# dpfried/action-segmentation

Measured on AMD Instinct MI355X. Metric: frames/sec semi-Markov decode, CrossTask T~10k K~20 L=1024, 1/2/4/8 GPUs, higher is better.
Workload: dtype f64

## Files before the change

### action-segmentation_amd/_build.py

```python
import os
import shutil
import subprocess
from concurrent.futures import ThreadPoolExecutor

HERE = os.path.dirname(os.path.abspath(__file__))
CSRC = os.path.join(HERE, "csrc")
OBJ = os.path.join(CSRC, "_obj")
LIB = os.path.join(HERE, "libsmmdp.so")
SOURCES = ["smm_api.hip", "smm_emission.hip", "smm_viterbi.hip", "smm_chunk.hip", "smm_logz.hip", "smm_logz_bwd.hip", "smm_dense.hip",
           "smm_eval.hip", "smm_fit.hip", "smm_tables.hip", "smm_sample.hip", "smm_kbest.hip",
           "smm_entropy.hip", "smm_kl.hip", "smm_entropy_bwd.hip", "smm_mbr.hip", "smm_align.hip", "smm_align_opt.hip", "smm_align_logz.hip",
           "smm_align_opt_logz.hip", "smm_align_graph.hip", "smm_align_graph_logz.hip",
           "smm_align_graph_sample.hip", "smm_align_graph_entropy.hip", "smm_align_graph_kl.hip",
           "smm_align_graph_entropy_bwd.hip"]
HEADERS = ["smm_device.h", "smm_launch.h", "smm_align_tile.h", "smm_align_lse.h", "smm_align_graph.h", "smm_posterior.h", "smm_draw.h", "smm_plan_feedback.h", os.path.join("..", "..", "include", "smmdp.h")]
FLAGS = ["--offload-arch=gfx950", "-O3", "-ffp-contract=off", "-fPIC", "-std=c++17",
         "-mllvm", "-pragma-unroll-threshold=1048576", "-mllvm", "-unroll-threshold=1048576"]


UNIT_FLAGS = {"smm_viterbi.hip": ["-fno-honor-nans", "-DSMM_FMAX_BUILTIN"]}


def _extra_flags():
    return os.environ.get("SMM_DEV_FLAGS", "").split()


def _obj(src):
    return os.path.join(OBJ, os.path.splitext(src)[0] + ".o")


def _stale_obj(src, force):
    o = _obj(src)
    if force or not os.path.exists(o):
        return True
    t = os.path.getmtime(o)
    return any(os.path.getmtime(os.path.join(CSRC, f)) > t for f in [src] + HEADERS)


def stale():
    if not os.path.exists(LIB):
        return True
    t = os.path.getmtime(LIB)
    return any(os.path.getmtime(os.path.join(CSRC, f)) > t for f in SOURCES + HEADERS)


def build(force=False, verbose=False):
    if not force and not stale():
        return LIB
# ... 57 lines not shown
```

### action-segmentation_amd/_lib.py

```python
import ctypes
import os

HERE = os.path.dirname(os.path.abspath(__file__))
LIB_PATH = os.environ.get("SMM_LIB_PATH") or os.path.join(HERE, "libsmmdp.so")

SYMBOLS = [
    "smm_strerror", "smm_last_hip_error", "smm_version", "smm_device_count", "smm_workspace_bytes",
    "smm_error_word_offset", "smm_dp_timing_enable", "smm_dp_timing_read", "smm_dp_timing_read_tagged", "smm_band_frame_ns", "smm_time_split_plan",
    "smm_env_reload", "smm_release_cached_plans", "smm_cached_plan_bytes", "smm_plan_feedback_info", "smm_plan_feedback_plan",
    "smm_emission_f64", "smm_emission_bwd_f64", "smm_viterbi_f64", "smm_viterbi_f32", "smm_decode_f32", "smm_logz_f64", "smm_logz_bwd_f64",
    "smm_sample_f64", "smm_entropy_f64", "smm_kl_f64", "smm_kbest_workspace_bytes", "smm_kbest_f64",
    "smm_mbr_workspace_bytes", "smm_mbr_f64",
    "smm_align_workspace_bytes", "smm_align_f64", "smm_align_opt_workspace_bytes", "smm_align_opt_f64",
    "smm_align_graph_workspace_bytes", "smm_align_graph_f64",
    "smm_align_logz_workspace_bytes", "smm_align_logz_f64", "smm_align_logz_bwd_f64",
    "smm_align_opt_logz_workspace_bytes", "smm_align_opt_logz_f64", "smm_align_opt_logz_bwd_f64",
    "smm_align_graph_logz_workspace_bytes", "smm_align_graph_logz_f64", "smm_align_graph_logz_bwd_f64",
    "smm_align_graph_sample_f64", "smm_align_graph_entropy_f64", "smm_align_graph_kl_f64",
    "smm_entropy_bwd_scratch_bytes", "smm_entropy_bwd_f64", "smm_kl_bwd_f64",
    "smm_align_graph_entropy_bwd_scratch_bytes", "smm_align_graph_entropy_bwd_f64", "smm_align_graph_kl_bwd_f64",
    "smm_factor_tables_f64", "smm_factor_tables_bwd_f64",
    "smm_dense_workspace_bytes", "smm_dense_dp_f32", "smm_dense_marginals_f32",
    "smm_eval_workspace_bytes", "smm_eval_confusion_i64", "smm_eval_videos_i64",
    "smm_fit_workspace_bytes", "smm_fit_error_word_offset", "smm_fit_stats_f64",
]


class SmmShape(ctypes.Structure):
    _fields_ = [("b", ctypes.c_int32), ("d", ctypes.c_int32), ("n_groups", ctypes.c_int32),
                ("c_max", ctypes.c_int32), ("k_rows", ctypes.c_int32), ("t_max", ctypes.c_int32),
                ("flags", ctypes.c_int32), ("total_frames", ctypes.c_int64)]


class SmmPlanFeedbackInfo(ctypes.Structure):
    _fields_ = [("n_replans", ctypes.c_int32), ("n1_before", ctypes.c_int32), ("n1_after", ctypes.c_int32),
                ("n_videos", ctypes.c_int32), ("end_before_us", ctypes.c_double), ("end_after_us", ctypes.c_double),
                ("stamps", ctypes.POINTER(ctypes.c_uint64)), ("order", ctypes.POINTER(ctypes.c_int32))]


class SmmTablesShape(ctypes.Structure):
    _fields_ = [("n_classes", ctypes.c_int32), ("d", ctypes.c_int32), ("n_groups", ctypes.c_int32),
# ... 114 lines not shown
                                                                                         ctypes.c_void_p]
    lib.smm_error_word_offset.argtypes = [ctypes.POINTER(SmmShape)]
    lib.smm_kl_f64.restype = ctypes.c_int
    lib.smm_kl_f64.argtypes = [ctypes.POINTER(SmmShape)] + [ctypes.c_void_p] * 11 + [ctypes.c_void_p, ctypes.c_size_t] \
        + [ctypes.c_void_p] * 6 + [ctypes.c_void_p, ctypes.c_size_t] + [ctypes.c_void_p] * 3
    lib.smm_entropy_bwd_scratch_bytes.restype = ctypes.c_size_t
    lib.smm_entropy_bwd_scratch_bytes.argtypes = [ctypes.POINTER(SmmShape), ctypes.c_void_p]
    lib.smm_entropy_bwd_f64.restype = ctypes.c_int
    lib.smm_entropy_bwd_f64.argtypes = [ctypes.POINTER(SmmShape)] + [ctypes.c_void_p] * 17 + [ctypes.c_void_p, ctypes.c_size_t] \
        + [ctypes.c_void_p, ctypes.c_size_t, ctypes.c_void_p]
    lib.smm_kl_bwd_f64.restype = ctypes.c_int
    lib.smm_kl_bwd_f64.argtypes = [ctypes.POINTER(SmmShape)] + [ctypes.c_void_p] * 11 + [ctypes.c_void_p, ctypes.c_size_t] \
        + [ctypes.c_void_p] * 6 + [ctypes.c_void_p, ctypes.c_size_t, ctypes.c_int32] + [ctypes.c_void_p] * 6 \
        + [ctypes.c_void_p, ctypes.c_size_t, ctypes.c_void_p]
    lib.smm_align_graph_entropy_bwd_scratch_bytes.restype = ctypes.c_size_t
    lib.smm_align_graph_entropy_bwd_scratch_bytes.argtypes = [ctypes.POINTER(SmmShape), ctypes.c_void_p, ctypes.c_void_p]
    lib.smm_align_graph_entropy_bwd_f64.restype = ctypes.c_int
    lib.smm_align_graph_entropy_bwd_f64.argtypes = [ctypes.POINTER(SmmShape)] + [ctypes.c_void_p] * 21 \
        + [ctypes.c_void_p, ctypes.c_size_t] * 2 + [ctypes.c_void_p]
    lib.smm_align_graph_kl_bwd_f64.restype = ctypes.c_int
    lib.smm_align_graph_kl_bwd_f64.argtypes = [ctypes.POINTER(SmmShape)] + [ctypes.c_void_p] * 11 + [ctypes.c_void_p, ctypes.c_size_t] \
        + [ctypes.c_void_p] * 4 + [ctypes.c_void_p, ctypes.c_size_t] + [ctypes.c_void_p] * 4 + [ctypes.c_int32] \
        + [ctypes.c_void_p] * 6 + [ctypes.c_void_p, ctypes.c_size_t, ctypes.c_void_p]
    lib.smm_dp_timing_enable.restype = None
    lib.smm_dp_timing_enable.argtypes = [ctypes.c_int]
    lib.smm_dp_timing_read.restype = ctypes.c_int
    lib.smm_dp_timing_read.argtypes = [ctypes.POINTER(ctypes.c_float), ctypes.c_int]
    lib.smm_dp_timing_read_tagged.restype = ctypes.c_int
    lib.smm_dp_timing_read_tagged.argtypes = [ctypes.POINTER(ctypes.c_float), ctypes.POINTER(ctypes.c_int32), ctypes.c_int]
    lib.smm_band_frame_ns.restype = ctypes.c_double
    lib.smm_band_frame_ns.argtypes = [ctypes.c_int]
    lib.smm_time_split_plan.restype = ctypes.c_int
    lib.smm_time_split_plan.argtypes = [ctypes.POINTER(SmmShape)] + [ctypes.c_void_p] * 4 + [ctypes.c_int] + [ctypes.c_void_p] * 4 + [ctypes.c_int]
    lib.smm_env_reload.restype = None
    lib.smm_env_reload.argtypes = []
    lib.smm_release_cached_plans.restype = ctypes.c_size_t
    lib.smm_release_cached_plans.argtypes = []
    lib.smm_cached_plan_bytes.restype = ctypes.c_size_t
    lib.smm_cached_plan_bytes.argtypes = []
    lib.smm_plan_feedback_info.restype = ctypes.c_int
    lib.smm_plan_feedback_info.argtypes = [ctypes.POINTER(SmmPlanFeedbackInfo)]
    lib.smm_plan_feedback_plan.restype = ctypes.c_int
    lib.smm_plan_feedback_plan.argtypes = [ctypes.c_int, ctypes.c_int, ctypes.c_double] + [ctypes.c_void_p] * 3 + [ctypes.c_int, ctypes.c_int] \
        + [ctypes.c_void_p] * 4
    _lib = lib
    return lib


def reload_env():
    if _lib is not None:
        _lib.smm_env_reload()


def check(status):
    if status != 0:
        lib = load()
        msg = lib.smm_strerror(status).decode()
        if status == -4:
            msg += " (hipError %d)" % lib.smm_last_hip_error()
        raise SmmError("libsmmdp: %s" % msg)


def host_cores():
    import os
    env = os.environ.get('SMM_HOST_CORES')
    if env:
# ... 17 lines not shown
```

### action-segmentation_amd/csrc/smm_api.hip

```cpp
#include <algorithm>
#include <atomic>
#include <functional>
#include <cstdio>
#include <cstdlib>
#include <cstring>
#include <numeric>
#include <vector>
#include <unordered_map>
#include <mutex>
#include <utility>
#include <string>

#include "../../include/smmdp.h"
#include "smm_device.h"
#include "smm_launch.h"
#include "smm_plan_feedback.h"

static thread_local int g_last_hip = 0;

namespace {
struct SmmEnv {
    int spec = 1;
    int no_split = 0;
    double split_min_us = 100.0, split_ns = 0.0;
    int split_margin = 400;
    int plan_cache = 1;
    int small_wg = 1;
    int plan_feedback = 1;
    int chunk = 1;
    int chunk_p = 0;
    int chunk_lmin = 0;
    int chunk_wc = 512;
    int no_bt_window = 0;
    int fit_grid = 0;
    int verbose = 0;
#ifdef SMM_DEV
    int debug_flags = 0;
    int split_debug = 0;
    int upload_memcpy = 0;
    int emission_v2 = 0;
#endif
    std::string key;
};
std::atomic<const SmmEnv *> g_env{nullptr};
std::once_flag g_env_once;

void env_read()
{
    SmmEnv e;
    struct Item { const char *name; int *i; double *d; };
    const Item items[] = {
        {"SMM_SPEC", &e.spec, nullptr}, {"SMM_NO_SPLIT", &e.no_split, nullptr}, {"SMM_SPLIT_MIN_US", nullptr, &e.split_min_us},
        {"SMM_SPLIT_NS", nullptr, &e.split_ns}, {"SMM_SPLIT_MARGIN", &e.split_margin, nullptr},
        {"SMM_PLAN_CACHE", &e.plan_cache, nullptr}, {"SMM_SMALL_WG", &e.small_wg, nullptr}, {"SMM_PLAN_FEEDBACK", &e.plan_feedback, nullptr}, {"SMM_CHUNK", &e.chunk, nullptr}, {"SMM_CHUNK_P", &e.chunk_p, nullptr},
        {"SMM_CHUNK_WC", &e.chunk_wc, nullptr}, {"SMM_CHUNK_LMIN", &e.chunk_lmin, nullptr}, {"SMM_NO_BT_WINDOW", &e.no_bt_window, nullptr},
        {"SMM_FIT_GRID", &e.fit_grid, nullptr}, {"SMM_VERBOSE", &e.verbose, nullptr},
#ifdef SMM_DEV
        {"SMM_DEBUG_FLAGS", &e.debug_flags, nullptr}, {"SMM_SPLIT_DEBUG", &e.split_debug, nullptr},
        {"SMM_UPLOAD_MEMCPY", &e.upload_memcpy, nullptr}, {"SMM_EMISSION_V2", &e.emission_v2, nullptr},
#endif
    };
    for (const Item &it : items) {
        const char *v = std::getenv(it.name);
        if (!v) continue;
        if (it.i) *it.i = (*v == 0) ? 1 : std::atoi(v);
        if (it.d) *it.d = std::atof(v);
        e.key += it.name; e.key += '='; e.key += v; e.key += ';';
    }
    g_env.store(new SmmEnv(e), std::memory_order_release);
}
const SmmEnv &env()
{
    std::call_once(g_env_once, env_read);
    return *g_env.load(std::memory_order_acquire);
}
}

extern "C" void smm_env_reload(void)
{
    (void)env();
    env_read();
}
int smm_env_fit_grid() { return env().fit_grid; }
int smm_env_emission_v2()
{
#ifdef SMM_DEV
    return env().emission_v2;
#else
// ... 235 lines not shown
    SmmChunkVideo *cvs;
    int32_t *redo;
    double *anchors;
    int n_cv, n_units, u_part1;
    int small_first, small_count;
    uint64_t *stamps = nullptr;
    hipEvent_t done = nullptr;
    void *fb_entry = nullptr;
    std::vector<int32_t> order_host, frames_host;
};

static bool band_mode(int kp_max, int c_need);

static int device_cus()
{
    static std::mutex mu;
    static int n_cu[64] = {};
    int dev = 0;
    if (hipGetDevice(&dev) != hipSuccess || dev < 0 || dev >= 64) return 0;
    std::lock_guard<std::mutex> lock(mu);
    if (!n_cu[dev] && hipDeviceGetAttribute(&n_cu[dev], hipDeviceAttributeMultiprocessorCount, dev) != hipSuccess) n_cu[dev] = 0;
    return n_cu[dev] > 0 ? n_cu[dev] : 0;
}

constexpr double SMM_BAND_NS_BASE = 145.0, SMM_BAND_NS_PER_STATE = 2.0;
extern "C" double smm_band_frame_ns(int n_states)
{
    if (n_states < 1 || n_states > SMM_MAX_STATES) return 0.0;
    return SMM_BAND_NS_BASE + SMM_BAND_NS_PER_STATE * n_states;
}

static double dp_frame_ns(bool band, int c) { return band ? smm_band_frame_ns(c) : 150.0 + 3.0 * c; }

static int choose_split(const SmmVideo *hv, int32_t *order, int b, int d, int c_max, int64_t total_frames)
{
    const SmmEnv &ev = env();
    if (b < 24 || ev.no_split) return 0;
    const int n_cu = device_cus();
    if (n_cu <= 0) return 0;
    const double em_us = (double)total_frames * (4.0 * d + 8.0 * c_max) / 4.0e6;
    if (em_us < ev.split_min_us) return 0;
    int tmax = 0;
    for (int i = 0; i < b; ++i) tmax = std::max(tmax, hv[i].T);
    const double split_ns = ev.split_ns > 0.0 ? ev.split_ns : 1.75 * smm_band_frame_ns(std::min(c_max, (int)SMM_MAX_STATES));
    const int thr = tmax - (int)(em_us * 1000.0 / split_ns) - ev.split_margin;
    int n1 = 0;
    for (int i = 0; i < b; ++i) n1 += hv[i].T >= thr;
    if (thr <= 0 || n1 < 1 || n1 > b / 3 || n1 > n_cu / 2 || b - n1 < 16 || b > 2 * n_cu) return 0;
    std::stable_partition(order, order + b, [&](int32_t v) { return hv[v].T >= thr; });
    return n1;
}

namespace {
struct PlanFeedback {
    uint64_t *stamps = nullptr;
    hipEvent_t done = nullptr;
    bool pending = false;
    bool have = false;
    bool busy = false;
    int evals_left = 5, n_replans = 0;
    int b = 0, n1_first = 0;
    double em_us = 0.0, end_before_us = 0.0, end_after_us = 0.0;
    std::vector<uint64_t> snap, used;
    std::vector<int32_t> order, frames;
};
constexpr int SMM_FEEDBACK_MAX_REPLANS = 4;
constexpr double SMM_FEEDBACK_MIN_GAIN = 0.02;
struct PlanEntry {
    PlanFeedback *fb = nullptr;
    std::vector<char> key;
    int device = 0;
// ... 372 lines not shown
}

extern "C" int smm_plan_feedback_info(smm_plan_feedback_info_t *out)
{
    if (!out) return SMM_ERR_ARG;
    std::lock_guard<std::mutex> lock(g_plans.mu);
    *out = g_fb_info.generation == g_plans.generation ? g_fb_info.info : smm_plan_feedback_info_t{};
    return SMM_OK;
}

extern "C" int smm_plan_feedback_plan(int b, int n_cu, double em_us, const double *dur_us, const int32_t *frames,
                                      const int32_t *cur_order, int cur_n1, int force, int32_t *order_out, int32_t *n1_out,
                                      double *end_current_us, double *end_chosen_us)
{
    if (b < 1 || n_cu < 1 || !dur_us || !frames || !cur_order || cur_n1 < 0 || cur_n1 > b) return SMM_ERR_ARG;
    std::vector<char> seen(b, 0);
    for (int i = 0; i < b; ++i) {
        if (cur_order[i] < 0 || cur_order[i] >= b || seen[cur_order[i]]) return SMM_ERR_ARG;
        seen[cur_order[i]] = 1;
    }
    const SmmFeedbackPlan p = smm_feedback_plan(dur_us, frames, cur_order, b, cur_n1, n_cu, em_us, force != 0);
    if (order_out) std::memcpy(order_out, p.order.data(), sizeof(int32_t) * b);
    if (n1_out) *n1_out = p.n1;
    if (end_current_us) *end_current_us = p.end_current_us;
    if (end_chosen_us) *end_chosen_us = p.end_chosen_us;
    return p.changed ? 1 : 0;
}

struct ChunkPlan {
    std::vector<SmmVideo> units;
    std::vector<SmmChunkVideo> cvs;
};

static void plan_chunks_lmin(const smm_shape *s, const SmmVideo *hv, const int32_t *n_states, int kp_max, bool band, ChunkPlan &out, int n_cu_given, int lmin_cfg)
{
    const SmmEnv &ev = env();
    if (!ev.chunk || (s->flags & (SMM_SHAPE_NO_EOS | SMM_SHAPE_NO_TIME_SPLIT)) || kp_max <= 64) return;
    const int n_cu = n_cu_given > 0 ? n_cu_given : device_cus();
    if (n_cu <= 0) return;
    auto ns = [&](int c) { return dp_frame_ns(band, c); };
    double t_cu = 0.0, t_long = 0.0;
    for (int i = 0; i < s->b; ++i) {
        const double t = (double)hv[i].T * ns(n_states[hv[i].group]);
        t_cu += t;
        t_long = std::max(t_long, t);
    }
    t_cu = t_cu / n_cu + (s->d > 0 ? (double)s->total_frames * (4.0 * s->d + 8.0 * s->c_max) / 4.0e3 : 0.0);
    if (ev.chunk_p <= 0 && t_long < 1.5 * t_cu) return;
    const size_t units_cap = chunk_units_max(s);
    for (int i = 0; i < s->b; ++i) {
        const int T = hv[i].T, C = n_states[hv[i].group], kpv = hv[i].kp;
        const int ov = std::max(std::min(ev.chunk_wc, kpv), 16) + kpv - 1;
        const int lmin = std::max(kpv - 1, std::min(lmin_cfg, 2 * kpv));
        const int pmin = ov + lmin;
        int P = ev.chunk_p > 0 ? ev.chunk_p : (int)(1.1 * t_cu / ns(C));
        P = std::max(P, pmin);
        if ((double)T < 1.05 * P || T < pmin + lmin) continue;
        int n_rest = (T - P + (P - ov) - 1) / (P - ov);
        int Pq = 0;
        for (; n_rest >= 1; --n_rest) {
            Pq = (int)(((int64_t)T + (int64_t)n_rest * ov + n_rest) / (n_rest + 1));
            if (Pq - ov >= lmin) break;
        }
        if (n_rest < 1 || n_rest + 1 > SMM_CHUNK_MAX_UNITS) continue;
        const int L = Pq - ov;
        size_t need = (size_t)3 * C * ((size_t)Pq + 1);
        for (int j = 1; j <= n_rest; ++j) {
            const int r = Pq + (j - 1) * L, e = (j == n_rest) ? T : r + L;
            need += (size_t)3 * C * ((size_t)(e - (r - ov)) + 1);
        }
        if (need > (size_t)8 * s->c_max * ((size_t)T + 1) || Pq + (n_rest - 1) * L >= T) continue;
        if (out.units.size() + n_rest + 1 > units_cap) break;
        SmmChunkVideo cv{i, (int32_t)out.units.size(), n_rest + 1, ov};
        size_t hoff = (size_t)hv[i].hist_off;
        for (int j = 0; j <= n_rest; ++j) {
            const int r = j ? Pq + (j - 1) * L : 0, a0 = j ? r - ov : 0, e = (j == n_rest) ? T : Pq + j * L;
            SmmVideo u = hv[i];
            u.frame_off = hv[i].frame_off + a0;
            u.hist_off = (int64_t)hoff;
            u.T = e - a0;
            u.pad = 1 | (j ? 2 : 0) | (a0 << 2);
            hoff += (size_t)3 * C * ((size_t)u.T + 1);
            out.units.push_back(u);
        }
        out.cvs.push_back(cv);
    }
}

static void plan_chunks(const smm_shape *s, const SmmVideo *hv, const int32_t *n_states, int kp_max, bool band, ChunkPlan &out, int n_cu_given = 0)
{
    const SmmEnv &ev = env();
    if (ev.chunk_lmin > 0) { plan_chunks_lmin(s, hv, n_states, kp_max, band, out, n_cu_given, std::max(ev.chunk_lmin, 130)); return; }
    const int n_cu = n_cu_given > 0 ? n_cu_given : device_cus();
    ChunkPlan fine;
    plan_chunks_lmin(s, hv, n_states, kp_max, band, fine, n_cu_given, SMM_CHUNK_LMIN_FINE);
    if (!fine.cvs.empty() && (int)fine.units.size() + (s->b - (int)fine.cvs.size()) <= n_cu) { out = std::move(fine); return; }
    plan_chunks_lmin(s, hv, n_states, kp_max, band, out, n_cu_given, SMM_CHUNK_LMIN);
}

static int stage_uncached(const smm_shape *s, const int64_t *lengths, const int64_t *frame_off, const int32_t *group,
                          const int32_t *kp, const int32_t *n_states, void *ws, size_t ws_bytes, hipStream_t stream, Staged *out,
                          bool for_viterbi, int cum_chunk, bool want_split, const std::function<char *(size_t)> *meta_alloc,
                          SmmPlan *plan_out)
{
    if (!shape_ok(s) || !lengths || !frame_off || !n_states || !ws) return SMM_ERR_ARG;
    if (!limits_ok(s)) return SMM_ERR_UNSUPPORTED;
    int c_need = 0;
    for (int g = 0; g < s->n_groups; ++g) {
        if (n_states[g] < 1 || n_states[g] > s->c_max) return SMM_ERR_ARG;
        c_need = std::max(c_need, n_states[g]);
    }
    const bool no_eos = (s->flags & SMM_SHAPE_NO_EOS) != 0;
    for (int i = 0; i < s->b; ++i)
        if (lengths[i] < (no_eos ? 2 : 1) || lengths[i] > s->t_max) return SMM_ERR_ARG;
    const SmmPlan p = make_plan(s, lengths);
    if (ws_bytes < p.total) return SMM_ERR_WORKSPACE;

    std::vector<char> host(p.meta_bytes, 0);
    SmmVideo *hv = reinterpret_cast<SmmVideo *>(host.data());
    int32_t *ho = reinterpret_cast<int32_t *>(host.data() + p.o_order);
    int32_t *hn = reinterpret_cast<int32_t *>(host.data() + p.o_nstates);

    size_t hoff = 0;
    int kp_max = 2;
    for (int i = 0; i < s->b; ++i) {
        const int64_t t = lengths[i];
        if (frame_off[i] < 0 || frame_off[i] + t > s->total_frames) return SMM_ERR_ARG;
        const int g = group ? group[i] : 0;
        if (g < 0 || g >= s->n_groups) return SMM_ERR_ARG;
        const int k = kp ? kp[i] : std::min<int>(s->k_rows, s->t_max);
        if (k < 1 || k > s->k_rows) return SMM_ERR_ARG;
        hv[i].frame_off = frame_off[i];
        hv[i].hist_off = (int64_t)hoff;
        hv[i].T = (int32_t)t;
        hv[i].group = g;
        hv[i].kp = k;
        hv[i].pad = 0;
        hoff += 8 * (size_t)s->c_max * (size_t)(t + 1);
        kp_max = std::max(kp_max, k);
    }
    std::iota(ho, ho + s->b, 0);
    out->band_mode = band_mode(kp_max, c_need);
    const bool band = out->band_mode;
    std::stable_sort(ho, ho + s->b, [&](int a, int b) {
        return hv[a].T * dp_frame_ns(band, n_states[hv[a].group]) > hv[b].T * dp_frame_ns(band, n_states[hv[b].group]);
    });
    if (cum_chunk > 0) std::stable_sort(ho, ho + s->b, [&](int a, int b) { return hv[a].group < hv[b].group; });
    std::memcpy(hn, n_states, sizeof(int32_t) * s->n_groups);
    ChunkPlan cp;
    if (for_viterbi && cum_chunk == 0) plan_chunks(s, hv, n_states, kp_max, out->band_mode, cp);
    const int n_cv = (int)cp.cvs.size(), n_un = (int)cp.units.size();
    out->n_cv = n_cv;
    out->n_units = s->b - n_cv + n_un;
    out->u_part1 = n_un;
    out->n_split = 0;
    if (n_cv > 0) {
        std::vector<char> is_cv(s->b, 0);
        for (const SmmChunkVideo &cv : cp.cvs) is_cv[cv.vid] = 1;
        std::stable_partition(ho, ho + s->b, [&](int32_t v) { return is_cv[v] != 0; });
        const SmmEnv &ev = env();
        const double em_us = (double)s->total_frames * (4.0 * s->d + 8.0 * s->c_max) / 4.0e6;
        if (want_split && !ev.no_split && s->b - n_cv >= 16 && em_us >= ev.split_min_us) out->n_split = n_cv;
    } else {
        out->n_split = want_split ? choose_split(hv, ho, s->b, s->d, s->c_max, s->total_frames) : 0;
    }
    out->small_first = out->small_count = 0;
    if (for_viterbi && cum_chunk == 0 && out->band_mode && env().small_wg && !(s->flags & SMM_SHAPE_NO_EOS)) {
        const bool force = env().small_wg >= 2;
        const int n_cu = device_cus();
        const int t0 = out->n_split > 0 ? out->n_split : n_cv;
        const int n_tail = s->b - t0;
        if (n_cu > 0 && (force || n_tail >= 3 * n_cu)) {
            double t_cu = 0.0;
            for (int i = t0; i < s->b; ++i) t_cu += (double)hv[ho[i]].T * smm_band_frame_ns(n_states[hv[ho[i]].group]);
            t_cu /= n_cu;
            auto small = [&](int32_t v) {
                return n_states[hv[v].group] <= 16 && (force || (double)hv[v].T * 1.6 * smm_band_frame_ns(n_states[hv[v].group]) <= 0.5 * t_cu);
            };
            const int n_small = (int)std::count_if(ho + t0, ho + s->b, small);
            if (n_small >= (force ? 1 : 64)) {
                std::stable_partition(ho + t0, ho + s->b, [&](int32_t v) { return !small(v); });
                out->small_count = n_small;
            }
// ... 41 lines not shown
            xp[i] = cp.cvs[i].vid;
        }
    }

    if (out->small_count > 0) out->small_first = out->n_units - out->small_count;

    char *base = static_cast<char *>(ws);
    const size_t o_ext = align_up(p.o_err, 256);
    char *meta_dst = meta_alloc ? (*meta_alloc)(o_ext + ext.size()) : nullptr;
    char *meta = meta_dst ? meta_dst : base;
    SMM_HIP((hipError_t)smm_upload_meta(meta, host.data(), p.o_err, stream));
    SMM_HIP((hipError_t)smm_zero_async(base + p.o_err, p.meta_bytes - p.o_err, stream));
    out->videos = reinterpret_cast<SmmVideo *>(meta);
    out->order = reinterpret_cast<int32_t *>(meta + p.o_order);
    out->n_states = reinterpret_cast<int32_t *>(meta + p.o_nstates);
    out->em_cum = reinterpret_cast<int32_t *>(meta + p.o_emcum);
    plan_point(p, ws, out);
    out->uvideos = nullptr; out->uorder = nullptr; out->porder = nullptr; out->cvs = nullptr;
    if (n_cv > 0) {
        char *xdst = meta_dst ? meta_dst + o_ext
                              : base + p.o_chunk + align_up(sizeof(int32_t) * s->b, 256) + align_up(sizeof(double) * chunk_units_max(s) * s->c_max, 256);
        SMM_HIP((hipError_t)smm_upload_meta(xdst, ext.data(), ext.size(), stream));
        out->uvideos = reinterpret_cast<SmmVideo *>(xdst);
        out->uorder = reinterpret_cast<int32_t *>(xdst + x_order);
        out->cvs = reinterpret_cast<SmmChunkVideo *>(xdst + x_cvs);
        out->porder = reinterpret_cast<int32_t *>(xdst + x_porder);
    }
    out->kp_max = kp_max;
    out->c_need = c_need;
    if (plan_out) *plan_out = p;
    return SMM_OK;
}

extern "C" int smm_time_split_plan(const smm_shape *s, const int64_t *lengths, const int32_t *group, const int32_t *kp,
                                   const int32_t *n_states, int n_cu, int32_t *unit_video, int32_t *unit_first, int32_t *unit_len,
                                   int32_t *unit_overlap, int cap)
{
    if (!shape_ok(s) || !lengths || !n_states || n_cu < 1) return SMM_ERR_ARG;
    std::vector<SmmVideo> hv(s->b);
    size_t hoff = 0;
    int kp_max = 2, c_need = 0;
    for (int g = 0; g < s->n_groups; ++g) c_need = std::max(c_need, n_states[g]);
    for (int i = 0; i < s->b; ++i) {
        const int g = group ? group[i] : 0;
        if (g < 0 || g >= s->n_groups || lengths[i] < 1) return SMM_ERR_ARG;
        hv[i] = SmmVideo{0, (int64_t)hoff, (int32_t)lengths[i], g, kp ? kp[i] : std::min<int>(s->k_rows, s->t_max), 0};
        hoff += 8 * (size_t)s->c_max * (size_t)(lengths[i] + 1);
        kp_max = std::max(kp_max, hv[i].kp);
    }
    ChunkPlan cp;
    plan_chunks(s, hv.data(), n_states, kp_max, band_mode(kp_max, c_need), cp, n_cu);
    int n = 0;
    for (const SmmChunkVideo &cv : cp.cvs)
        for (int j = 0; j < cv.n_chunks; ++j, ++n) {
            if (n >= cap) continue;
            const SmmVideo &u = cp.units[cv.first_unit + j];
            if (unit_video) unit_video[n] = cv.vid;
            if (unit_first) unit_first[n] = u.pad >> 2;
            if (unit_len) unit_len[n] = u.T;
            if (unit_overlap) unit_overlap[n] = j ? cv.ov : 0;
        }
    return n;
}

static bool band_mode(int kp_max, int c_need)
{
    return kp_max > 512 || (kp_max > 256 && c_need > 28);
}

static int ring_regs(int kp_max)
{
    int r = 1;
    while (64 * r < kp_max) r *= 2;
    return r;
}

struct Tables {
    const double *elp, *trans, *init, *len, *endpen, *logz;
};

static SmmDpArgs dp_args(const smm_shape *s, const Staged &st, const Tables &t)
{
    SmmDpArgs a{};
    a.videos = st.videos; a.order = st.order; a.n_states = st.n_states;
    a.elp = t.elp; a.trans = t.trans; a.init = t.init; a.len = t.len; a.endpen = t.endpen;
    a.hist = st.hist; a.err = st.err;
    a.c_max = s->c_max; a.k_rows = s->k_rows; a.t_max = s->t_max; a.b = s->b;
    if (s->flags & SMM_SHAPE_NO_EOS) { a.flags |= 8; a.endpen = nullptr; }
    return a;
}

static SmmPostHead post_head(const smm_shape *s, const Staged &st)
{
    return {st.videos, st.n_states, st.err, s->c_max, s->k_rows, s->b, (s->flags & SMM_SHAPE_NO_EOS) ? 1 : 0};
// ... 1401 lines not shown
```

### action-segmentation_amd/ops.py

```python
import ctypes

import numpy as np
import torch

from . import _lib
from ._lib import SmmShape


class Batch:

    def __init__(self, lengths, n_states, k_rows, c_max=None, frame_offset=None, group=None, kp=None, d=0,
                 t_max=None, total_frames=None, no_eos=False, no_time_split=False):
        self.lengths = np.ascontiguousarray(np.asarray(lengths, dtype=np.int64).reshape(-1))
        self.b = int(self.lengths.shape[0])
        self.n_states = np.ascontiguousarray(np.asarray(n_states, dtype=np.int32).reshape(-1))
        self.n_groups = int(self.n_states.shape[0])
        self.c_max = int(c_max if c_max is not None else self.n_states.max())
        self.k_rows = int(k_rows)
        self.t_max = int(t_max if t_max is not None else self.lengths.max())
        if frame_offset is None:
            frame_offset = np.arange(self.b, dtype=np.int64) * self.t_max
        self.frame_offset = np.ascontiguousarray(np.asarray(frame_offset, dtype=np.int64).reshape(-1))
        self.group = None if group is None else np.ascontiguousarray(np.asarray(group, dtype=np.int32).reshape(-1))
        self.kp = None if kp is None else np.ascontiguousarray(np.asarray(kp, dtype=np.int32).reshape(-1))
# ... 1202 lines not shown
def plan_feedback_plan(dur_us, frames, cur_order, cur_n1, n_cu, em_us, force=False):
    import numpy as np
    dur = np.ascontiguousarray(dur_us, dtype=np.float64)
    fr = np.ascontiguousarray(frames, dtype=np.int32)
    cur = np.ascontiguousarray(cur_order, dtype=np.int32)
    b = len(dur)
    if len(fr) != b or len(cur) != b:
        raise ValueError("dur_us, frames and cur_order must have one entry per video")
    order = np.zeros(b, dtype=np.int32)
    n1 = ctypes.c_int32(0)
    e0, e1 = ctypes.c_double(0.0), ctypes.c_double(0.0)
    ptr = lambda a: ctypes.c_void_p(a.ctypes.data)
    rc = _lib.load().smm_plan_feedback_plan(b, int(n_cu), float(em_us), ptr(dur), ptr(fr), ptr(cur), int(cur_n1), 1 if force else 0,
                                            ptr(order), ctypes.cast(ctypes.byref(n1), ctypes.c_void_p),
                                            ctypes.cast(ctypes.byref(e0), ctypes.c_void_p), ctypes.cast(ctypes.byref(e1), ctypes.c_void_p))
    if rc < 0:
        _lib.check(rc)
    return bool(rc), order, int(n1.value), float(e0.value), float(e1.value)


def time_split_plan(batch, n_cu=256):
    import numpy as np
    lib = _lib.load()
    ln, fo, gr, kp, ns = batch.host_ptrs()
    cap = int(batch.total_frames // 128 + 2 * batch.b + 8)
    arrs = [np.zeros(cap, dtype=np.int32) for _ in range(4)]
    n = lib.smm_time_split_plan(ctypes.byref(batch.shape), ctypes.c_void_p(ln), ctypes.c_void_p(gr), ctypes.c_void_p(kp), ctypes.c_void_p(ns),
                                int(n_cu), *[ctypes.c_void_p(a.ctypes.data) for a in arrs], cap)
    if n < 0:
        raise _lib.SmmError("smm_time_split_plan: %s" % lib.smm_strerror(n).decode())
    return [tuple(int(a[i]) for a in arrs) for i in range(min(n, cap))]


def reload_env():
    _lib.reload_env()


def release_cached_plans():
    torch.cuda.synchronize()
    return int(_lib.load().smm_release_cached_plans())


def cached_plan_bytes():
    return int(_lib.load().smm_cached_plan_bytes())
```

### include/smmdp.h

```cpp
#ifndef SMMDP_H
#define SMMDP_H

#include <stddef.h>
#include <stdint.h>

#ifdef __cplusplus
extern "C" {
#endif

typedef enum smm_status {
    SMM_OK = 0,
    SMM_ERR_ARG = -1,
    SMM_ERR_UNSUPPORTED = -2,
    SMM_ERR_WORKSPACE = -3,
    SMM_ERR_HIP = -4,
    SMM_ERR_NO_DEVICE = -5
} smm_status;

#define SMM_MAX_STATES 32
#define SMM_MAX_K_ROWS 1024

typedef struct smm_shape {
    int32_t b;
    int32_t d;
    int32_t n_groups;
    int32_t c_max;
    int32_t k_rows;
    int32_t t_max;
    int32_t flags;
    int64_t total_frames;
} smm_shape;

#define SMM_SHAPE_NO_EOS 1
#define SMM_SHAPE_LOGZ_BOTH 2
#define SMM_SHAPE_NO_TIME_SPLIT 4

const char *smm_strerror(int status);
int smm_last_hip_error(void);
const char *smm_version(void);
int smm_device_count(void);

size_t smm_workspace_bytes(const smm_shape *shape, const int64_t *lengths_host);

size_t smm_error_word_offset(const smm_shape *shape);


int smm_time_split_plan(const smm_shape *shape, const int64_t *lengths_host, const int32_t *group_host, const int32_t *kp_host,
                        const int32_t *n_states_host, int n_cu, int32_t *unit_video, int32_t *unit_first, int32_t *unit_len,
                        int32_t *unit_overlap, int cap);

void smm_dp_timing_enable(int on);
int smm_dp_timing_read(float *ms, int cap);
int smm_dp_timing_read_tagged(float *ms, int32_t *tags, int cap);

double smm_band_frame_ns(int n_states);

size_t smm_release_cached_plans(void);
size_t smm_cached_plan_bytes(void);
void smm_env_reload(void);

typedef struct smm_plan_feedback_info_t {
    int32_t n_replans;
    int32_t n1_before, n1_after;
    int32_t n_videos;
    double end_before_us;
    double end_after_us;
    const uint64_t *stamps;
    const int32_t *order;
} smm_plan_feedback_info_t;
int smm_plan_feedback_info(smm_plan_feedback_info_t *out);

int smm_plan_feedback_plan(int b, int n_cu, double em_us, const double *dur_us, const int32_t *frames, const int32_t *cur_order,
                           int cur_n1, int force, int32_t *order_out, int32_t *n1_out, double *end_current_us,
                           double *end_chosen_us);

int smm_emission_f64(const smm_shape *shape, const int64_t *lengths_host, const int64_t *frame_offset_host,
                     const int32_t *group_host, const int32_t *n_states_host,
                     const float *x, const double *w, const double *cst, const double *inv_var, const float *cons,
                     double *elp64, float *elp32, void *workspace, size_t workspace_bytes, void *stream);

int smm_emission_bwd_f64(const smm_shape *shape, const int64_t *lengths_host, const int64_t *frame_offset_host,
                         const int32_t *group_host, const int32_t *n_states_host,
// ... 293 lines not shown
```

Before: 1.003 billion.

## Split longest videos into two time chunks using a replay cost model

Adds a host-side replay scheduler model that estimates the batch makespan when the S longest videos are each split into two overlapping time units. It picks the S with the best modelled end time and adopts the split only if the model predicts a sufficient gain. The plan is used in the Viterbi staging path when no regular chunk plan fires. The aim is to shorten the tail where a few long videos run alone on single CUs after the rest finish. In exchange it adds planning overhead, stitching work and overlap recomputation, and depends on hand-tuned model constants.

```diff
diff --git a/action-segmentation_amd/_build.py b/action-segmentation_amd/_build.py
--- a/action-segmentation_amd/_build.py
+++ b/action-segmentation_amd/_build.py
@@ -13,7 +13,7 @@
            "smm_align_opt_logz.hip", "smm_align_graph.hip", "smm_align_graph_logz.hip",
            "smm_align_graph_sample.hip", "smm_align_graph_entropy.hip", "smm_align_graph_kl.hip",
            "smm_align_graph_entropy_bwd.hip"]
-HEADERS = ["smm_device.h", "smm_launch.h", "smm_align_tile.h", "smm_align_lse.h", "smm_align_graph.h", "smm_posterior.h", "smm_draw.h", "smm_plan_feedback.h", os.path.join("..", "..", "include", "smmdp.h")]
+HEADERS = ["smm_device.h", "smm_launch.h", "smm_align_tile.h", "smm_align_lse.h", "smm_align_graph.h", "smm_posterior.h", "smm_draw.h", "smm_plan_feedback.h", "smm_split_replay.h", os.path.join("..", "..", "include", "smmdp.h")]
 FLAGS = ["--offload-arch=gfx950", "-O3", "-ffp-contract=off", "-fPIC", "-std=c++17",
          "-mllvm", "-pragma-unroll-threshold=1048576", "-mllvm", "-unroll-threshold=1048576"]
 
diff --git a/action-segmentation_amd/_lib.py b/action-segmentation_amd/_lib.py
--- a/action-segmentation_amd/_lib.py
+++ b/action-segmentation_amd/_lib.py
@@ -7,6 +7,7 @@
 SYMBOLS = [
     "smm_strerror", "smm_last_hip_error", "smm_version", "smm_device_count", "smm_workspace_bytes",
     "smm_error_word_offset", "smm_dp_timing_enable", "smm_dp_timing_read", "smm_dp_timing_read_tagged", "smm_band_frame_ns", "smm_time_split_plan",
+    "smm_decode_split_plan",
     "smm_env_reload", "smm_release_cached_plans", "smm_cached_plan_bytes", "smm_plan_feedback_info", "smm_plan_feedback_plan",
     "smm_emission_f64", "smm_emission_bwd_f64", "smm_viterbi_f64", "smm_viterbi_f32", "smm_decode_f32", "smm_logz_f64", "smm_logz_bwd_f64",
     "smm_sample_f64", "smm_entropy_f64", "smm_kl_f64", "smm_kbest_workspace_bytes", "smm_kbest_f64",
@@ -187,6 +188,8 @@
     lib.smm_band_frame_ns.argtypes = [ctypes.c_int]
     lib.smm_time_split_plan.restype = ctypes.c_int
     lib.smm_time_split_plan.argtypes = [ctypes.POINTER(SmmShape)] + [ctypes.c_void_p] * 4 + [ctypes.c_int] + [ctypes.c_void_p] * 4 + [ctypes.c_int]
+    lib.smm_decode_split_plan.restype = ctypes.c_int
+    lib.smm_decode_split_plan.argtypes = lib.smm_time_split_plan.argtypes + [ctypes.c_void_p] * 3 + [ctypes.c_int]
     lib.smm_env_reload.restype = None
     lib.smm_env_reload.argtypes = []
     lib.smm_release_cached_plans.restype = ctypes.c_size_t
diff --git a/action-segmentation_amd/csrc/smm_api.hip b/action-segmentation_amd/csrc/smm_api.hip
--- a/action-segmentation_amd/csrc/smm_api.hip
+++ b/action-segmentation_amd/csrc/smm_api.hip
@@ -15,6 +15,7 @@
 #include "smm_device.h"
 #include "smm_launch.h"
 #include "smm_plan_feedback.h"
+#include "smm_split_replay.h"
 
 static thread_local int g_last_hip = 0;
 
@@ -31,6 +32,7 @@
     int chunk_p = 0;
     int chunk_lmin = 0;
     int chunk_wc = 512;
+    int chunk_replay = 1;
     int no_bt_window = 0;
     int fit_grid = 0;
     int verbose = 0;
@@ -53,7 +55,7 @@
         {"SMM_SPEC", &e.spec, nullptr}, {"SMM_NO_SPLIT", &e.no_split, nullptr}, {"SMM_SPLIT_MIN_US", nullptr, &e.split_min_us},
         {"SMM_SPLIT_NS", nullptr, &e.split_ns}, {"SMM_SPLIT_MARGIN", &e.split_margin, nullptr},
         {"SMM_PLAN_CACHE", &e.plan_cache, nullptr}, {"SMM_SMALL_WG", &e.small_wg, nullptr}, {"SMM_PLAN_FEEDBACK", &e.plan_feedback, nullptr}, {"SMM_CHUNK", &e.chunk, nullptr}, {"SMM_CHUNK_P", &e.chunk_p, nullptr},
-        {"SMM_CHUNK_WC", &e.chunk_wc, nullptr}, {"SMM_CHUNK_LMIN", &e.chunk_lmin, nullptr}, {"SMM_NO_BT_WINDOW", &e.no_bt_window, nullptr},
+        {"SMM_CHUNK_WC", &e.chunk_wc, nullptr}, {"SMM_CHUNK_LMIN", &e.chunk_lmin, nullptr}, {"SMM_CHUNK_REPLAY", &e.chunk_replay, nullptr}, {"SMM_NO_BT_WINDOW", &e.no_bt_window, nullptr},
         {"SMM_FIT_GRID", &e.fit_grid, nullptr}, {"SMM_VERBOSE", &e.verbose, nullptr},
 #ifdef SMM_DEV
         {"SMM_DEBUG_FLAGS", &e.debug_flags, nullptr}, {"SMM_SPLIT_DEBUG", &e.split_debug, nullptr},
@@ -355,11 +357,11 @@
 
 static double dp_frame_ns(bool band, int c) { return band ? smm_band_frame_ns(c) : 150.0 + 3.0 * c; }
 
-static int choose_split(const SmmVideo *hv, int32_t *order, int b, int d, int c_max, int64_t total_frames)
+static int choose_split(const SmmVideo *hv, int32_t *order, int b, int d, int c_max, int64_t total_frames, int n_cu_given = 0)
 {
     const SmmEnv &ev = env();
     if (b < 24 || ev.no_split) return 0;
-    const int n_cu = device_cus();
+    const int n_cu = n_cu_given > 0 ? n_cu_given : device_cus();
     if (n_cu <= 0) return 0;
     const double em_us = (double)total_frames * (4.0 * d + 8.0 * c_max) / 4.0e6;
     if (em_us < ev.split_min_us) return 0;
@@ -798,7 +800,8 @@
     std::vector<SmmChunkVideo> cvs;
 };
 
-static void plan_chunks_lmin(const smm_shape *s, const SmmVideo *hv, const int32_t *n_states, int kp_max, bool band, ChunkPlan &out, int n_cu_given, int lmin_cfg)
+static void plan_chunks_lmin(const smm_shape *s, const SmmVideo *hv, const int32_t *n_states, int kp_max, bool band, ChunkPlan &out, int n_cu_given, int lmin_cfg,
+                             const char *two_units = nullptr)
 {
     const SmmEnv &ev = env();
     if (!ev.chunk || (s->flags & (SMM_SHAPE_NO_EOS | SMM_SHAPE_NO_TIME_SPLIT)) || kp_max <= 64) return;
@@ -812,17 +815,18 @@
         t_long = std::max(t_long, t);
     }
     t_cu = t_cu / n_cu + (s->d > 0 ? (double)s->total_frames * (4.0 * s->d + 8.0 * s->c_max) / 4.0e3 : 0.0);
-    if (ev.chunk_p <= 0 && t_long < 1.5 * t_cu) return;
+    if (!two_units && ev.chunk_p <= 0 && t_long < 1.5 * t_cu) return;
     const size_t units_cap = chunk_units_max(s);
     for (int i = 0; i < s->b; ++i) {
         const int T = hv[i].T, C = n_states[hv[i].group], kpv = hv[i].kp;
         const int ov = std::max(std::min(ev.chunk_wc, kpv), 16) + kpv - 1;
         const int lmin = std::max(kpv - 1, std::min(lmin_cfg, 2 * kpv));
         const int pmin = ov + lmin;
-        int P = ev.chunk_p > 0 ? ev.chunk_p : (int)(1.1 * t_cu / ns(C));
+        if (two_units && !two_units[i]) continue;
+        int P = two_units ? pmin : ev.chunk_p > 0 ? ev.chunk_p : (int)(1.1 * t_cu / ns(C));
         P = std::max(P, pmin);
         if ((double)T < 1.05 * P || T < pmin + lmin) continue;
-        int n_rest = (T - P + (P - ov) - 1) / (P - ov);
+        int n_rest = two_units ? 1 : (T - P + (P - ov) - 1) / (P - ov);
         int Pq = 0;
         for (; n_rest >= 1; --n_rest) {
             Pq = (int)(((int64_t)T + (int64_t)n_rest * ov + n_rest) / (n_rest + 1));
@@ -853,15 +857,62 @@
     }
 }
 
-static void plan_chunks(const smm_shape *s, const SmmVideo *hv, const int32_t *n_states, int kp_max, bool band, ChunkPlan &out, int n_cu_given = 0)
+struct DecodeSplitInfo {
+    SmmSplitReplay replay;
+    int unsplit_n1 = 0;
+};
+static void plan_chunks_replay(const smm_shape *s, const SmmVideo *hv, const int32_t *n_states, int kp_max, bool band, ChunkPlan &out, int n_cu_given,
+                               const int32_t *decode_order, DecodeSplitInfo *info);
+
+static void plan_chunks(const smm_shape *s, const SmmVideo *hv, const int32_t *n_states, int kp_max, bool band, ChunkPlan &out, int n_cu_given = 0,
+                        const int32_t *decode_order = nullptr, DecodeSplitInfo *info = nullptr)
 {
     const SmmEnv &ev = env();
     if (ev.chunk_lmin > 0) { plan_chunks_lmin(s, hv, n_states, kp_max, band, out, n_cu_given, std::max(ev.chunk_lmin, 130)); return; }
     const int n_cu = n_cu_given > 0 ? n_cu_given : device_cus();
+    if (decode_order && ev.chunk_replay >= 2 && ev.chunk_p <= 0) {
+        plan_chunks_replay(s, hv, n_states, kp_max, band, out, n_cu_given, decode_order, info);
+        if (!out.cvs.empty()) return;
+    }
     ChunkPlan fine;
     plan_chunks_lmin(s, hv, n_states, kp_max, band, fine, n_cu_given, SMM_CHUNK_LMIN_FINE);
     if (!fine.cvs.empty() && (int)fine.units.size() + (s->b - (int)fine.cvs.size()) <= n_cu) { out = std::move(fine); return; }
     plan_chunks_lmin(s, hv, n_states, kp_max, band, out, n_cu_given, SMM_CHUNK_LMIN);
+    if (out.cvs.empty() && decode_order && ev.chunk_p <= 0) plan_chunks_replay(s, hv, n_states, kp_max, band, out, n_cu_given, decode_order, info);
+}
+
+static void plan_chunks_replay(const smm_shape *s, const SmmVideo *hv, const int32_t *n_states, int kp_max, bool band, ChunkPlan &out, int n_cu_given,
+                               const int32_t *decode_order, DecodeSplitInfo *info)
+{
+    const SmmEnv &ev = env();
+    if (!ev.chunk || !ev.chunk_replay || (s->flags & (SMM_SHAPE_NO_EOS | SMM_SHAPE_NO_TIME_SPLIT)) || kp_max <= 64) return;
+    const int n_cu = n_cu_given > 0 ? n_cu_given : device_cus();
+    if (n_cu <= 0) return;
+    const int b = s->b;
+    std::vector<int32_t> unsplit(decode_order, decode_order + b);
+    const int n1 = choose_split(hv, unsplit.data(), b, s->d, s->c_max, s->total_frames, n_cu);
+    if (info) info->unsplit_n1 = n1;
+    if (n1 < 1) return;
+    std::vector<double> dur(b);
+    std::vector<int32_t> frames(b), kp(b);
+    for (int i = 0; i < b; ++i) {
+        frames[i] = hv[i].T;
+        kp[i] = hv[i].kp;
+        dur[i] = 1e-3 * (double)hv[i].T * dp_frame_ns(band, n_states[hv[i].group]);
+    }
+    SmmSplitReplayModel m;
+    m.warmup = ev.chunk_wc;
+    m.lmin = SMM_CHUNK_LMIN;
+    const double em_us = (double)s->total_frames * (4.0 * s->d + 8.0 * s->c_max) / 4.0e6;
+    SmmSplitReplay r = smm_split_replay_plan(dur.data(), frames.data(), kp.data(), unsplit.data(), b, n1, n_cu, em_us, m);
+    if (ev.chunk_replay >= 2) r.s_adopted = std::min(ev.chunk_replay, r.s_max);
+    if (r.s_adopted > 0) {
+        std::vector<char> two(b, 0);
+        for (int i = 0; i < r.s_adopted; ++i) two[r.by_time[i]] = 1;
+        plan_chunks_lmin(s, hv, n_states, kp_max, band, out, n_cu, SMM_CHUNK_LMIN, two.data());
+        if ((int)out.cvs.size() != r.s_adopted || (int)out.units.size() != 2 * r.s_adopted) { out = ChunkPlan(); r.s_adopted = 0; }
+    }
+    if (info) info->replay = std::move(r);
 }
 
 static int stage_uncached(const smm_shape *s, const int64_t *lengths, const int64_t *frame_off, const int32_t *group,
@@ -914,7 +965,7 @@
     if (cum_chunk > 0) std::stable_sort(ho, ho + s->b, [&](int a, int b) { return hv[a].group < hv[b].group; });
     std::memcpy(hn, n_states, sizeof(int32_t) * s->n_groups);
     ChunkPlan cp;
-    if (for_viterbi && cum_chunk == 0) plan_chunks(s, hv, n_states, kp_max, out->band_mode, cp);
+    if (for_viterbi && cum_chunk == 0) plan_chunks(s, hv, n_states, kp_max, out->band_mode, cp, 0, want_split ? ho : nullptr);
     const int n_cv = (int)cp.cvs.size(), n_un = (int)cp.units.size();
     out->n_cv = n_cv;
     out->n_units = s->b - n_cv + n_un;
@@ -1022,9 +1073,9 @@
     return SMM_OK;
 }
 
-extern "C" int smm_time_split_plan(const smm_shape *s, const int64_t *lengths, const int32_t *group, const int32_t *kp,
-                                   const int32_t *n_states, int n_cu, int32_t *unit_video, int32_t *unit_first, int32_t *unit_len,
-                                   int32_t *unit_overlap, int cap)
+static int time_split_plan(const smm_shape *s, const int64_t *lengths, const int32_t *group, const int32_t *kp,
+                           const int32_t *n_states, int n_cu, int32_t *unit_video, int32_t *unit_first, int32_t *unit_len,
+                           int32_t *unit_overlap, int cap, bool decode, DecodeSplitInfo *info)
 {
     if (!shape_ok(s) || !lengths || !n_states || n_cu < 1) return SMM_ERR_ARG;
     std::vector<SmmVideo> hv(s->b);
@@ -1039,7 +1090,16 @@
         kp_max = std::max(kp_max, hv[i].kp);
     }
     ChunkPlan cp;
-    plan_chunks(s, hv.data(), n_states, kp_max, band_mode(kp_max, c_need), cp, n_cu);
+    const bool band = band_mode(kp_max, c_need);
+    std::vector<int32_t> order;
+    if (decode) {
+        order.resize(s->b);
+        std::iota(order.begin(), order.end(), 0);
+        std::stable_sort(order.begin(), order.end(), [&](int a, int b) {
+            return hv[a].T * dp_frame_ns(band, n_states[hv[a].group]) > hv[b].T * dp_frame_ns(band, n_states[hv[b].group]);
+        });
+    }
+    plan_chunks(s, hv.data(), n_states, kp_max, band, cp, n_cu, decode ? order.data() : nullptr, info);
     int n = 0;
     for (const SmmChunkVideo &cv : cp.cvs)
         for (int j = 0; j < cv.n_chunks; ++j, ++n) {
@@ -1050,6 +1110,30 @@
             if (unit_len) unit_len[n] = u.T;
             if (unit_overlap) unit_overlap[n] = j ? cv.ov : 0;
         }
+    return n;
+}
+
+extern "C" int smm_time_split_plan(const smm_shape *s, const int64_t *lengths, const int32_t *group, const int32_t *kp,
+                                   const int32_t *n_states, int n_cu, int32_t *unit_video, int32_t *unit_first, int32_t *unit_len,
+                                   int32_t *unit_overlap, int cap)
+{
+    return time_split_plan(s, lengths, group, kp, n_states, n_cu, unit_video, unit_first, unit_len, unit_overlap, cap, false, nullptr);
+}
+
+extern "C" int smm_decode_split_plan(const smm_shape *s, const int64_t *lengths, const int32_t *group, const int32_t *kp,
+                                     const int32_t *n_states, int n_cu, int32_t *unit_video, int32_t *unit_first, int32_t *unit_len,
+                                     int32_t *unit_overlap, int cap, int32_t *s_info, double *end_us, double *end_by_s, int end_cap)
+{
+    if (s && s->n_groups > 0 && n_states)
+        for (int g = 0; g < s->n_groups; ++g)
+            if (n_states[g] < 1 || n_states[g] > s->c_max) return SMM_ERR_ARG;
+    DecodeSplitInfo info;
+    const int n = time_split_plan(s, lengths, group, kp, n_states, n_cu, unit_video, unit_first, unit_len, unit_overlap, cap, true, &info);
+    if (n < 0) return n;
+    const SmmSplitReplay &r = info.replay;
+    if (s_info) { s_info[0] = r.s_adopted; s_info[1] = r.s_best; s_info[2] = r.s_max; s_info[3] = info.unsplit_n1; }
+    if (end_us) { end_us[0] = r.end_unsplit_us; end_us[1] = r.end_best_us; end_us[2] = r.end_replanned_us; }
+    for (int i = 0; end_by_s && i < end_cap; ++i) end_by_s[i] = i < (int)r.end_us.size() ? r.end_us[i] : 0.0;
     return n;
 }
 
diff --git a/action-segmentation_amd/csrc/smm_split_replay.h b/action-segmentation_amd/csrc/smm_split_replay.h
--- /dev/null
+++ b/action-segmentation_amd/csrc/smm_split_replay.h
@@ -0,0 +1,128 @@
+#pragma once
+#include <algorithm>
+#include <cstdint>
+#include <functional>
+#include <numeric>
+#include <queue>
+#include <vector>
+
+#include "smm_plan_feedback.h"
+
+struct SmmSplitReplayModel {
+    int warmup = 512;
+    int lmin = 512;
+    double pfx_fixed_us = 8.3, pfx_row_ns = 6.6;
+    double stitch_seg_us = 2.0, stitch_seg_frames = 48.0;
+    double dp_scale = 0.87, em_scale = 1.15;
+    double unit_slow = 1.15;
+    double min_gain = 0.05;
+    int min_rest = 16;
+};
+
+struct SmmSplitReplay {
+    std::vector<int32_t> by_time;
+    std::vector<double> end_us;
+    int s_max = 0;
+    int s_best = 0;
+    int s_adopted = 0;
+    double end_best_us = 0.0;
+    double end_unsplit_us = 0.0;
+    double end_replanned_us = 0.0;
+};
+
+inline bool smm_split_two_units(int T, int kp, const SmmSplitReplayModel &m, int *first_len, int *second_first, int *second_len)
+{
+    if (T < 1 || kp < 1) return false;
+    const int64_t ov = (int64_t)std::max(std::min(m.warmup, kp), 16) + kp - 1;
+    const int64_t lmin = std::max<int64_t>(kp - 1, std::min<int64_t>(m.lmin, 2 * (int64_t)kp));
+    if ((int64_t)T < ov + 2 * lmin) return false;
+    const int64_t pq = ((int64_t)T + ov + 1) / 2;
+    if (pq - ov < lmin || pq >= T) return false;
+    if (first_len) *first_len = (int)pq;
+    if (second_first) *second_first = (int)(pq - ov);
+    if (second_len) *second_len = (int)(T - (pq - ov));
+    return true;
+}
+
+inline double smm_split_stitch_us(int T, const SmmSplitReplayModel &m)
+{
+    return m.stitch_seg_frames > 0.0 ? m.stitch_seg_us * (double)T / m.stitch_seg_frames : 0.0;
+}
+
+inline double smm_split_replay_end(const double *dur_us, const int32_t *frames, const int32_t *kp, const int32_t *by_time, int b, int S,
+                                   int n_cu, double em_us, const SmmSplitReplayModel &m)
+{
+    if (b < 1 || S < 1 || S >= b || n_cu < 1 || 2 * (int64_t)S > n_cu) return 0.0;
+    double f1 = 0.0, f_all = 0.0;
+    for (int i = 0; i < b; ++i) {
+        f_all += (double)frames[by_time[i]];
+        if (i < S) f1 += (double)frames[by_time[i]];
+    }
+    const double em1 = f_all > 0.0 ? em_us * f1 / f_all : 0.0;
+    int rows = 0;
+    for (int i = 0; i < S; ++i) {
+        const int v = by_time[i];
+        int second_first = 0;
+        if (!smm_split_two_units(frames[v], kp[v], m, nullptr, &second_first, nullptr)) return 0.0;
+        rows = std::max(rows, second_first);
+    }
+    const double t_units = em1 + m.pfx_fixed_us + 1e-3 * m.pfx_row_ns * rows;
+    std::vector<double> free_at;
+    free_at.reserve(n_cu);
+    double t_dp = t_units;
+    for (int i = 0; i < S; ++i) {
+        const int v = by_time[i];
+        int first_len = 0, second_len = 0;
+        smm_split_two_units(frames[v], kp[v], m, &first_len, nullptr, &second_len);
+        const double per_pos = frames[v] > 0 ? m.unit_slow * dur_us[v] / (double)frames[v] : 0.0;
+        for (const int len : {first_len, second_len}) {
+            const double e = t_units + per_pos * len;
+            t_dp = std::max(t_dp, e);
+            free_at.push_back(std::max(e, em_us));
+        }
+    }
+    while ((int)free_at.size() < n_cu) free_at.push_back(em_us);
+    std::priority_queue<double, std::vector<double>, std::greater<double>> cus(std::greater<double>(), std::move(free_at));
+    double end = t_dp;
+    int rest = S, stitch = 0;
+    while (rest < b || stitch < S) {
+        const double f = cus.top();
+        cus.pop();
+        double e;
+        if (stitch < S && (rest >= b || f >= t_dp)) e = std::max(f, t_dp) + smm_split_stitch_us(frames[by_time[stitch++]], m);
+        else e = f + dur_us[by_time[rest++]];
+        cus.push(e);
+        end = std::max(end, e);
+    }
+    return end;
+}
+
+inline SmmSplitReplay smm_split_replay_plan(const double *model_us, const int32_t *frames, const int32_t *kp, const int32_t *unsplit_order,
+                                            int b, int unsplit_n1, int n_cu, double em_model_us, const SmmSplitReplayModel &m = SmmSplitReplayModel())
+{
+    SmmSplitReplay out;
+    if (b < 1 || n_cu < 1 || unsplit_n1 < 1) return out;
+    std::vector<double> dur(model_us, model_us + b);
+    for (double &d : dur) d *= m.dp_scale;
+    const double *dur_us = dur.data();
+    const double em_us = em_model_us * m.em_scale;
+    out.end_unsplit_us = smm_feedback_replay(dur_us, frames, unsplit_order, b, unsplit_n1, n_cu, em_us);
+    if (!(out.end_unsplit_us > 0.0)) return out;
+    out.end_replanned_us = smm_feedback_plan(dur_us, frames, unsplit_order, b, unsplit_n1, n_cu, em_us).end_chosen_us;
+    out.by_time.assign(unsplit_order, unsplit_order + b);
+    std::stable_sort(out.by_time.begin(), out.by_time.end(), [&](int32_t x, int32_t y) { return dur_us[x] > dur_us[y]; });
+    const int cap = std::min(n_cu / 2, b - m.min_rest);
+    while (out.s_max < cap) {
+        const int v = out.by_time[out.s_max];
+        if (!smm_split_two_units(frames[v], kp[v], m, nullptr, nullptr, nullptr)) break;
+        ++out.s_max;
+    }
+    out.end_us.assign((size_t)out.s_max + 1, 0.0);
+    for (int S = 1; S <= out.s_max; ++S) {
+        const double e = smm_split_replay_end(dur_us, frames, kp, out.by_time.data(), b, S, n_cu, em_us, m);
+        out.end_us[S] = e;
+        if (e > 0.0 && (out.s_best == 0 || e < out.end_best_us)) { out.s_best = S; out.end_best_us = e; }
+    }
+    if (out.s_best > 0 && out.end_best_us <= (1.0 - m.min_gain) * out.end_unsplit_us) out.s_adopted = out.s_best;
+    return out;
+}
diff --git a/action-segmentation_amd/ops.py b/action-segmentation_amd/ops.py
--- a/action-segmentation_amd/ops.py
+++ b/action-segmentation_amd/ops.py
@@ -1258,6 +1258,23 @@
     return [tuple(int(a[i]) for a in arrs) for i in range(min(n, cap))]
 
 
+def decode_split_plan(batch, n_cu=256):
+    import numpy as np
+    lib = _lib.load()
+    ln, fo, gr, kp, ns = batch.host_ptrs()
+    cap = int(batch.total_frames // 128 + 2 * batch.b + 8)
+    arrs = [np.zeros(cap, dtype=np.int32) for _ in range(4)]
+    s_info, ends, by_s = np.zeros(4, dtype=np.int32), np.zeros(3), np.zeros(batch.b + 1)
+    ptr = lambda a: ctypes.c_void_p(a.ctypes.data)
+    n = lib.smm_decode_split_plan(ctypes.byref(batch.shape), ctypes.c_void_p(ln), ctypes.c_void_p(gr), ctypes.c_void_p(kp), ctypes.c_void_p(ns),
+                                  int(n_cu), *[ptr(a) for a in arrs], cap, ptr(s_info), ptr(ends), ptr(by_s), len(by_s))
+    if n < 0:
+        raise _lib.SmmError("smm_decode_split_plan: %s" % lib.smm_strerror(n).decode())
+    return {'units': [tuple(int(a[i]) for a in arrs) for i in range(min(n, cap))], 's': int(s_info[0]), 's_best': int(s_info[1]),
+            's_max': int(s_info[2]), 'unsplit_n1': int(s_info[3]), 'end_unsplit_us': float(ends[0]), 'end_best_us': float(ends[1]), 'end_replanned_us': float(ends[2]),
+            'end_by_s': by_s[:int(s_info[2]) + 1].copy()}
+
+
 def reload_env():
     _lib.reload_env()
 
diff --git a/include/smmdp.h b/include/smmdp.h
--- a/include/smmdp.h
+++ b/include/smmdp.h
@@ -48,6 +48,10 @@
 int smm_time_split_plan(const smm_shape *shape, const int64_t *lengths_host, const int32_t *group_host, const int32_t *kp_host,
                         const int32_t *n_states_host, int n_cu, int32_t *unit_video, int32_t *unit_first, int32_t *unit_len,
                         int32_t *unit_overlap, int cap);
+
+int smm_decode_split_plan(const smm_shape *shape, const int64_t *lengths_host, const int32_t *group_host, const int32_t *kp_host,
+                          const int32_t *n_states_host, int n_cu, int32_t *unit_video, int32_t *unit_first, int32_t *unit_len,
+                          int32_t *unit_overlap, int cap, int32_t *s_info, double *end_us, double *end_by_s, int end_cap);
 
 void smm_dp_timing_enable(int on);
 int smm_dp_timing_read(float *ms, int cap);
```

Result: no change. 1.001 billion (-0.2%).
